# godk1122/IsaacLab

Hardware: AMD Instinct MI355X
Metric: env-steps/sec (whole node), Anymal-C rough 4096 envs/GPU, RSL-RL PPO iteration (collect+GAE+update) (higher is better)
Workload: dtype f32; 1 GPU; Isaac-Velocity-Rough-Anymal-C-v0, 4096 envs/GPU, T=24, 5 epochs x 4 minibatches, terrain 1204008 triangles, 4 state snapshots resident in HBM; parallelism=dp1, rollout=hipGraph, full_step=False, update=hipGraph (measured eager 16.24 ms, graph 15.60 ms), policy_params=571801

## Files before the change

### include/imx.h

```cpp
#ifndef IMX_H_
#define IMX_H_

#include <stddef.h>
#include <stdint.h>

#ifdef __cplusplus
extern "C" {
#endif

typedef struct imx_plan imx_plan_t;
typedef struct imx_mesh imx_mesh_t;
typedef void* imx_stream_t;

#define IMX_MAGIC 0x31584D49
#define IMX_PLAN_VERSION 3
#define IMX_HEADER_WORDS 48
#define IMX_MAX_OBS_GROUPS 4
#define IMX_REC_WORDS 20
#define IMX_FRAME_WORDS 9
#define IMX_FT_HEADER_WORDS 4

enum imx_header_word {
    IMX_H_MAGIC = 0, IMX_H_VERSION, IMX_H_J, IMX_H_B, IMX_H_H, IMX_H_A, IMX_H_D, IMX_H_R, IMX_H_NTERM, IMX_H_NREW,
    IMX_H_NOBS, IMX_H_NACT, IMX_H_MAX_EP_LEN, IMX_H_STEP_DT , IMX_H_TERM_OFF, IMX_H_REW_OFF, IMX_H_OBS_OFF,
// ... 514 lines not shown
size_t imx_empirical_normalization_partials_bytes(int64_t N, int64_t D);
int imx_empirical_normalization_update(int ngroups, const imx_norm_group_t* groups, imx_stream_t stream);


size_t imx_mlp_scratch_bytes(int64_t M, int out_features, int in_features);

int imx_mlp_dw(int64_t M, int N, int K, const float* dY_d, int64_t ldy, const float* X_d, int64_t ldx, float* dW_d,
               float* db_d, void* scratch_d, size_t scratch_bytes, imx_stream_t stream);

typedef struct imx_reduce_batch imx_reduce_batch_t;
int imx_reduce_batch_create(imx_reduce_batch_t** out);
void imx_reduce_batch_destroy(imx_reduce_batch_t* batch);
int imx_mlp_set_dw_cu_budget(int cus);
int imx_reduce_batch_begin(imx_reduce_batch_t* batch);
int imx_reduce_batch_flush(imx_reduce_batch_t* batch, imx_stream_t stream);

int imx_mlp_dw_elu(int64_t M, int N, int K, const float* dH_d, int64_t ldg, const float* H_d, int64_t ldh, float elu_alpha,
                   float* dZ_out_d, int64_t ldd, const float* X_d, int64_t ldx, float* dW_d, float* db_d, void* scratch_d,
                   size_t scratch_bytes, imx_stream_t stream);

int imx_mlp_infer(int64_t M, const float* X_d, int64_t ldx, int nnets, const int* nlayers, const int* dims,
                  const float* const* weights_d, const int* weight_pitch, const float* const* biases_d, const float* elu_alpha,
                  float* const* out_d, imx_stream_t stream);

typedef struct imx_policy_act {
    const float* std_d;
    uint64_t seed;
    const int32_t* step_counter_d;
    float* actions_out_d;
    float* logp_out_d;
    float* mu_out_d;
    float* sigma_out_d;
    float* obs_out_d;
    const imx_plan_t* plan;
// ... 126 lines not shown
```

### isaaclab_amd/csrc/mlp.hip

```cpp
#include <algorithm>

#include "imx_internal.h"
#include "imx_infer_device.h"


namespace {

constexpr int DW_T = 128;
constexpr int DW_BM = 32;
constexpr int DW_LD = DW_T + 32;

struct DwArgs {
    int64_t M;
    int N, K;
    const float* dY;
    int64_t ldy;
    const float* X;
    int64_t ldx;
    float* part;
    float* part_db;
    int tn, tk, S;
    int64_t rps;
    const float* H;
    int64_t ldh;
    float* Dout;
    int64_t ldd;
    float alpha;
};

template <bool VEC>
__device__ __forceinline__ void dw_load(float (&r)[16], const float* __restrict__ src, int64_t ld, int64_t row0, int64_t row_end,
                                        int col0, int ncols, int t) {
    if (VEC) {
        const int c = col0 + 4 * (t & 31);
        const int rr = t >> 5;
#pragma unroll
        for (int i = 0; i < 4; ++i) {
            const int64_t row = row0 + rr + 8 * i;
            float4 v = make_float4(0.f, 0.f, 0.f, 0.f);
            if (row < row_end && c < ncols) v = *reinterpret_cast<const float4*>(src + row * ld + c);
            r[4 * i] = v.x; r[4 * i + 1] = v.y; r[4 * i + 2] = v.z; r[4 * i + 3] = v.w;
        }
    } else {
        const int c = col0 + (t & 127);
        const int rr = t >> 7;
#pragma unroll
        for (int i = 0; i < 16; ++i) {
            const int64_t row = row0 + rr + 2 * i;
            r[i] = (row < row_end && c < ncols) ? src[row * ld + c] : 0.0f;
        }
    }
}

template <bool VEC>
__device__ __forceinline__ void dw_store(const float (&r)[16], float* __restrict__ s, int t) {
    if (VEC) {
        const int c = 4 * (t & 31), rr = t >> 5;
#pragma unroll
        for (int i = 0; i < 4; ++i)
            *reinterpret_cast<float4*>(s + (rr + 8 * i) * DW_LD + c) = make_float4(r[4 * i], r[4 * i + 1], r[4 * i + 2], r[4 * i + 3]);
    } else {
        const int c = t & 127, rr = t >> 7;
#pragma unroll
        for (int i = 0; i < 16; ++i) s[(rr + 2 * i) * DW_LD + c] = r[i];
    }
}

template <bool VEC>
__device__ __forceinline__ void dw_store_global(const float (&r)[16], float* __restrict__ dst, int64_t ld, int64_t row0, int64_t row_end,
                                                int col0, int ncols, int t, unsigned groups) {
    if (VEC) {
        const int c = col0 + 4 * (t & 31);
#pragma unroll
        for (int i = 0; i < 4; ++i) {
            const int64_t row = row0 + (t >> 5) + 8 * i;
            if (((groups >> i) & 1u) && row < row_end && c < ncols)
                *reinterpret_cast<float4*>(dst + row * ld + c) = make_float4(r[4 * i], r[4 * i + 1], r[4 * i + 2], r[4 * i + 3]);
        }
    } else {
// ... 1 lines not shown
#pragma unroll
        for (int i = 0; i < 16; ++i) {
            const int64_t row = row0 + (t >> 7) + 2 * i;
            if (row < row_end && c < ncols) dst[row * ld + c] = r[i];
        }
    }
}

typedef float dw_f4 __attribute__((ext_vector_type(4)));
typedef unsigned dw_u4 __attribute__((ext_vector_type(4)));

__device__ __forceinline__ __amdgpu_buffer_rsrc_t dw_rsrc(const float* p, int64_t rows, int64_t ld, int ncols) {
    return __builtin_amdgcn_make_buffer_rsrc(const_cast<float*>(p), 0, (int)(((rows - 1) * ld + ncols) * 4), 0x00020000);
}

template <bool ACT>
__device__ __forceinline__ void dw_movers_steady(const DwArgs& a, float* __restrict__ sY, float* __restrict__ sX, int t, int n0, int k0,
                                                 int64_t m_begin, int nst, bool want_db, unsigned dgroups, float (&dbv)[4]) {
    const int cl = 4 * (t & 31), rr = t >> 5;
    const int kv = (a.K + 3) & ~3;
    const int rows = nst * DW_BM;
    const int oy = (int)((rr * a.ldy + min(n0 + cl, a.N - 4)) * 4);
    const int ox = (int)((rr * a.ldx + min(k0 + cl, kv - 4)) * 4);
    const int oh = ACT ? (int)((rr * a.ldh + min(n0 + cl, a.N - 4)) * 4) : 0;
    const int od = ACT ? (int)((rr * a.ldd + n0 + cl) * 4) : 0;
    const bool d_ok = n0 + cl < a.N;
    const __amdgpu_buffer_rsrc_t by = dw_rsrc(a.dY + m_begin * a.ldy, rows, a.ldy, a.N);
    const __amdgpu_buffer_rsrc_t bx = dw_rsrc(a.X + m_begin * a.ldx, rows, a.ldx, kv);
    const __amdgpu_buffer_rsrc_t bh = dw_rsrc(ACT ? a.H + m_begin * a.ldh : a.dY, rows, ACT ? a.ldh : a.ldy, a.N);
    const __amdgpu_buffer_rsrc_t bd = dw_rsrc(ACT && dgroups != 0u ? a.Dout + m_begin * a.ldd : a.dY, rows, ACT ? a.ldd : a.ldy, a.N);
    const int gy = (int)(32 * a.ldy), gx = (int)(32 * a.ldx), gh = (int)(32 * a.ldh), gd = (int)(32 * a.ldd);
    int sy = 0, sx = 0, sh = 0, sd = 0;
    dw_f4 ry[4], rx[4], rh[ACT ? 4 : 1];
    auto load = [&]() __attribute__((always_inline)) {
#pragma unroll
        for (int i = 0; i < 4; ++i) ry[i] = __builtin_bit_cast(dw_f4, __builtin_amdgcn_raw_buffer_load_b128(by, oy, sy + i * gy, 0));
        if constexpr (ACT) {
#pragma unroll
            for (int i = 0; i < 4; ++i) rh[i] = __builtin_bit_cast(dw_f4, __builtin_amdgcn_raw_buffer_load_b128(bh, oh, sh + i * gh, 0));
            sh += 4 * gh;
        }
#pragma unroll
        for (int i = 0; i < 4; ++i) rx[i] = __builtin_bit_cast(dw_f4, __builtin_amdgcn_raw_buffer_load_b128(bx, ox, sx + i * gx, 0));
        sy += 4 * gy;
        sx += 4 * gx;
    };
    auto store = [&](int buf) __attribute__((always_inline)) {
        if constexpr (ACT) {
#pragma unroll
            for (int i = 0; i < 4; ++i)
#pragma unroll
                for (int j = 0; j < 4; ++j) ry[i][j] *= rh[i][j] > 0.0f ? 1.0f : rh[i][j] + a.alpha;
            if (dgroups != 0u) {
                if (d_ok) {
#pragma unroll
                    for (int i = 0; i < 4; ++i)
                        if ((dgroups >> i) & 1u) __builtin_amdgcn_raw_buffer_store_b128(__builtin_bit_cast(dw_u4, ry[i]), bd, od, sd + i * gd, 0);
                }
                sd += 4 * gd;
            }
        }
        float* py = sY + buf * (DW_BM * DW_LD) + rr * DW_LD + cl;
        float* px = sX + buf * (DW_BM * DW_LD) + rr * DW_LD + cl;
#pragma unroll
        for (int i = 0; i < 4; ++i) *reinterpret_cast<dw_f4*>(py + 8 * i * DW_LD) = ry[i];
#pragma unroll
        for (int i = 0; i < 4; ++i) *reinterpret_cast<dw_f4*>(px + 8 * i * DW_LD) = rx[i];
        if (want_db) {
#pragma unroll
            for (int i = 0; i < 4; ++i) { dbv[0] += ry[i][0]; dbv[1] += ry[i][1]; dbv[2] += ry[i][2]; dbv[3] += ry[i][3]; }
        }
    };
    load();
    store(0);
    if (nst > 1) load();
    __syncthreads();
    for (int st = 0; st < nst; ++st) {
        if (st + 1 < nst) {
            store((st + 1) & 1);
            if (st + 2 < nst) load();
        }
        __syncthreads();
    }
}

template <bool YVEC, bool XVEC, bool ACT>
__global__ void __launch_bounds__(512, 1) k_mlp_dw(DwArgs a) {
    __shared__ float sY[2][DW_BM * DW_LD];
    __shared__ float sX[2][DW_BM * DW_LD];
    const int T = a.tn * a.tk;
    int tile, s;
    if ((a.S & 7) == 0) {
        const int xcd = blockIdx.x & 7, j = blockIdx.x >> 3;
        tile = j % T;
        s = (j / T) * 8 + xcd;
    } else {
        tile = blockIdx.x % T;
        s = blockIdx.x / T;
    }
    const int n0 = (tile / a.tk) * DW_T, k0 = (tile % a.tk) * DW_T;
    const int64_t m_begin = (int64_t)s * a.rps, m_end = std::min<int64_t>(m_begin + a.rps, a.M);
    const int nst = (int)((m_end - m_begin + DW_BM - 1) / DW_BM);
    const bool want_db = a.part_db != nullptr && (tile % a.tk) == 0;

    if (threadIdx.x >= 256) {
        const int t = threadIdx.x - 256;
        float ry[16], rx[16], rh[ACT ? 16 : 1];
        float dbv[4] = {0.f, 0.f, 0.f, 0.f};
        int64_t loaded_row0 = 0;
        unsigned dgroups = 0u;
        if (ACT && a.Dout != nullptr) {
            if (YVEC) {
#pragma unroll
                for (int i = 0; i < 4; ++i) dgroups |= (i % a.tk) == (tile % a.tk) ? 1u << i : 0u;
            } else if ((tile % a.tk) == 0) {
                dgroups = 15u;
            }
        }
        const bool write_d = dgroups != 0u;
        bool steady = false;
        if constexpr (YVEC && XVEC) {
            int64_t ld = std::max(a.ldy, a.ldx);
            if (ACT) ld = std::max(ld, std::max(a.ldh, a.ldd));
            steady = nst > 0 && (m_end - m_begin) % DW_BM == 0 && a.rps * ld < ((int64_t)1 << 28);
            if (steady) dw_movers_steady<ACT>(a, &sY[0][0], &sX[0][0], t, n0, k0, m_begin, nst, want_db, dgroups, dbv);
        }
        auto load = [&](int st) {
            const int64_t row0 = m_begin + (int64_t)st * DW_BM;
            loaded_row0 = row0;
            dw_load<YVEC>(ry, a.dY, a.ldy, row0, m_end, n0, a.N, t);
            if constexpr (ACT) dw_load<YVEC>(rh, a.H, a.ldh, row0, m_end, n0, a.N, t);
            dw_load<XVEC>(rx, a.X, a.ldx, row0, m_end, k0, a.K, t);
        };
        auto store = [&](int buf) {
            if constexpr (ACT) {
#pragma unroll
                for (int q = 0; q < 16; ++q) ry[q] *= rh[q] > 0.0f ? 1.0f : rh[q] + a.alpha;
                if (write_d) dw_store_global<YVEC>(ry, a.Dout, a.ldd, loaded_row0, m_end, n0, a.N, t, dgroups);
            }
            dw_store<YVEC>(ry, sY[buf], t);
            dw_store<XVEC>(rx, sX[buf], t);
            if (want_db) {
                if (YVEC) {
#pragma unroll
                    for (int i = 0; i < 4; ++i) { dbv[0] += ry[4 * i]; dbv[1] += ry[4 * i + 1]; dbv[2] += ry[4 * i + 2]; dbv[3] += ry[4 * i + 3]; }
                } else {
#pragma unroll
                    for (int i = 0; i < 16; ++i) dbv[0] += ry[i];
                }
            }
        };
        if (!steady) {
            if (nst > 0) {
                load(0);
                store(0);
                if (nst > 1) load(1);
// ... 17 lines not shown
            }
        }
        __syncthreads();
        if (want_db && t < DW_T && n0 + t < a.N) {
            const float* red = sY[0];
            float sum = 0.0f;
            const int groups = YVEC ? 8 : 2;
            for (int g = 0; g < groups; ++g) sum += red[g * DW_T + t];
            a.part_db[(size_t)s * a.N + n0 + t] = sum;
        }
        return;
    }
    const int t = threadIdx.x;
    const int lane = t & 63, w = t >> 6, r = lane & 31, half = lane >> 5;
    const int wn = w & 1, wk = w >> 1;
    f32x16 acc[2][2];
#pragma unroll
    for (int i = 0; i < 2; ++i)
#pragma unroll
        for (int j = 0; j < 2; ++j)
#pragma unroll
            for (int q = 0; q < 16; ++q) acc[i][j][q] = 0.0f;
    __syncthreads();
    for (int st = 0; st < nst; ++st) {
        const float* py = sY[st & 1] + half * DW_LD + wn * 64 + r;
        const float* px = sX[st & 1] + half * DW_LD + wk * 64 + r;
        float p0 = py[0], p1 = py[32], p2 = px[0], p3 = px[32], q0, q1, q2, q3;
#pragma unroll
        for (int kk = 0; kk < DW_BM / 2; kk += 2) {
            q0 = py[(kk + 1) * 2 * DW_LD]; q1 = py[(kk + 1) * 2 * DW_LD + 32];
            q2 = px[(kk + 1) * 2 * DW_LD]; q3 = px[(kk + 1) * 2 * DW_LD + 32];
            __builtin_amdgcn_sched_barrier(0);
            acc[0][0] = __builtin_amdgcn_mfma_f32_32x32x2f32(p0, p2, acc[0][0], 0, 0, 0);
            acc[0][1] = __builtin_amdgcn_mfma_f32_32x32x2f32(p0, p3, acc[0][1], 0, 0, 0);
            acc[1][0] = __builtin_amdgcn_mfma_f32_32x32x2f32(p1, p2, acc[1][0], 0, 0, 0);
            acc[1][1] = __builtin_amdgcn_mfma_f32_32x32x2f32(p1, p3, acc[1][1], 0, 0, 0);
            __builtin_amdgcn_sched_barrier(0);
            if (kk + 2 < DW_BM / 2) {
                p0 = py[(kk + 2) * 2 * DW_LD]; p1 = py[(kk + 2) * 2 * DW_LD + 32];
                p2 = px[(kk + 2) * 2 * DW_LD]; p3 = px[(kk + 2) * 2 * DW_LD + 32];
            }
            __builtin_amdgcn_sched_barrier(0);
            acc[0][0] = __builtin_amdgcn_mfma_f32_32x32x2f32(q0, q2, acc[0][0], 0, 0, 0);
            acc[0][1] = __builtin_amdgcn_mfma_f32_32x32x2f32(q0, q3, acc[0][1], 0, 0, 0);
            acc[1][0] = __builtin_amdgcn_mfma_f32_32x32x2f32(q1, q2, acc[1][0], 0, 0, 0);
            acc[1][1] = __builtin_amdgcn_mfma_f32_32x32x2f32(q1, q3, acc[1][1], 0, 0, 0);
            __builtin_amdgcn_sched_barrier(0);
        }
        __syncthreads();
    }
    float* part = a.part + (size_t)s * a.N * a.K;
    const bool interior = n0 + DW_T <= a.N && k0 + DW_T <= a.K;
#pragma unroll
    for (int bi = 0; bi < 2; ++bi)
#pragma unroll
        for (int bj = 0; bj < 2; ++bj) {
            const int k = k0 + wk * 64 + bj * 32 + r;
            if (interior) {
#pragma unroll
                for (int q = 0; q < 16; ++q) part[(size_t)(n0 + wn * 64 + bi * 32 + acc_row(q, half)) * a.K + k] = acc[bi][bj][q];
            } else {
#pragma unroll
                for (int q = 0; q < 16; ++q) {
                    const int n = n0 + wn * 64 + bi * 32 + acc_row(q, half);
                    if (n < a.N && k < a.K) part[(size_t)n * a.K + k] = acc[bi][bj][q];
                }
            }
        }
    __syncthreads();
}

constexpr int RED_Y = 16;
__global__ void __launch_bounds__(64 * RED_Y) k_mlp_reduce(int64_t total, int S, const float* __restrict__ part, float* __restrict__ out,
                                                          int N, const float* __restrict__ part_db, float* __restrict__ db) {
    __shared__ float red[RED_Y][64];
    const int tx = threadIdx.x, ty = threadIdx.y;
    const int64_t i = (int64_t)blockIdx.x * 64 + tx;
    const float* src = nullptr;
    int64_t stride = 0;
    float* dst = nullptr;
    if (i < total) {
        src = part + i; stride = total; dst = out + i;
    } else if (db && i - total < N) {
        src = part_db + (i - total); stride = N; dst = db + (i - total);
// ... 78 lines not shown
        float sum = 0.0f;
#pragma unroll
        for (int y = 0; y < RED_Y; ++y) sum += red[y][tx];
        *dst = sum;
    }
}

struct DwPlan {
    int tn, tk, S;
    int64_t rps;
};

int g_num_cu = 0;
int g_dw_cu_budget = 0;

DwPlan dw_plan(int64_t M, int N, int K) {
    if (g_num_cu == 0) {
        int dev = 0, cu = 0;
        if (hipGetDevice(&dev) != hipSuccess || hipDeviceGetAttribute(&cu, hipDeviceAttributeMultiprocessorCount, dev) != hipSuccess || cu <= 0)
            cu = 256;
        g_num_cu = cu;
    }
    DwPlan p;
    p.tn = (N + DW_T - 1) / DW_T;
    p.tk = (K + DW_T - 1) / DW_T;
    const int T = p.tn * p.tk;
    const int cus = g_dw_cu_budget > 0 ? std::min(g_dw_cu_budget, g_num_cu) : g_num_cu;
    int64_t S = std::max<int64_t>(1, (int64_t)cus / T);
    S = std::min<int64_t>(S, std::max<int64_t>(1, M / (2 * DW_BM)));
    if (S >= 8) S &= ~(int64_t)7;
    p.rps = ((M + S - 1) / S + DW_BM - 1) / DW_BM * DW_BM;
    p.S = (int)((M + p.rps - 1) / p.rps);
    return p;
}

constexpr int HEAD_A = 64;

#define IMX_HALF_LOG_2PI_F 0.91893853320467274178f
template <bool ELU_IN, int AMAX, int LOSS>
__global__ void __launch_bounds__(256) k_head_fwd(int64_t M, int K, int A, float* __restrict__ h, int64_t ldh,
// ... 516 lines not shown
    return 0;
}

extern "C" void imx_reduce_batch_destroy(imx_reduce_batch_t* b) {
    if (t_batch == b) t_batch = nullptr;
    delete b;
}

extern "C" int imx_reduce_batch_begin(imx_reduce_batch_t* b) {
    IMX_REQUIRE(b, "imx_reduce_batch_begin: null batch");
    IMX_REQUIRE(t_batch == nullptr, "imx_reduce_batch_begin: another batch is still open on this thread (flush it first)");
    t_batch = b;
    return 0;
}

extern "C" int imx_reduce_batch_flush(imx_reduce_batch_t* b, imx_stream_t stream) {
    IMX_REQUIRE(b && t_batch == b, "imx_reduce_batch_flush: this batch is not the one open on this thread");
    t_batch = nullptr;
    if (b->args.n == 0) return 0;
    hipLaunchKernelGGL(k_mlp_reduce_batch, dim3(b->blocks), dim3(64, RED_Y), 0, (hipStream_t)stream, b->args);
    b->args.n = 0;
    b->blocks = 0;
    IMX_HIP(hipGetLastError());
    return 0;
}

extern "C" int imx_mlp_dw(int64_t M, int N, int K, const float* dY_d, int64_t ldy, const float* X_d, int64_t ldx, float* dW_d,
                          float* db_d, void* scratch_d, size_t scratch_bytes, imx_stream_t stream) {
    return mlp_dw_launch("imx_mlp_dw", M, N, K, dY_d, ldy, nullptr, 0, 0.0f, nullptr, 0, X_d, ldx, dW_d, db_d, scratch_d, scratch_bytes,
                         stream);
}

extern "C" int imx_mlp_dw_elu(int64_t M, int N, int K, const float* dH_d, int64_t ldg, const float* H_d, int64_t ldh, float elu_alpha,
                              float* dZ_out_d, int64_t ldd, const float* X_d, int64_t ldx, float* dW_d, float* db_d, void* scratch_d,
                              size_t scratch_bytes, imx_stream_t stream) {
    IMX_REQUIRE(H_d, "imx_mlp_dw_elu: the saved activation output is required");
    return mlp_dw_launch("imx_mlp_dw_elu", M, N, K, dH_d, ldg, H_d, ldh, elu_alpha, dZ_out_d, ldd, X_d, ldx, dW_d, db_d, scratch_d,
                         scratch_bytes, stream);
}

static int head_fwd_launch(int64_t M, int K, int A, float* h_d, int64_t ldh, const float* W_d, const float* b_d, float* y_d,
                           int elu_in_place, float elu_alpha, const imx_head_loss_t* loss, imx_stream_t stream) {
    IMX_REQUIRE(M > 0 && h_d && W_d && b_d && y_d, "imx_mlp_head_fwd: bad arguments");
    IMX_REQUIRE(A >= 1 && A <= HEAD_A, "imx_mlp_head_fwd: %d outputs (1..%d supported; wider layers are library GEMMs)", A, HEAD_A);
    IMX_REQUIRE(K >= 16 && K % 16 == 0 && K <= 2048 && ldh >= K && ldh % 4 == 0 && aligned16(h_d),
                "imx_mlp_head_fwd: in-features %d (pitch %lld) must be a multiple of 16, 16-byte aligned rows", K, (long long)ldh);
    IMX_REQUIRE((size_t)A * K * sizeof(float) <= 64 * 1024, "imx_mlp_head_fwd: %d x %d weights do not fit the 64 KB of LDS used", A, K);
    imx_head_loss_t L{};
    int mode = 0;
    if (loss) {
        L = *loss;
        mode = L.mode;
        IMX_REQUIRE(mode == 1 || mode == 2, "imx_mlp_head_fwd_loss: mode %d (1 policy, 2 value)", mode);
// ... 523 lines not shown
```

### isaaclab_amd/rsl_rl/ppo.py

```python

from __future__ import annotations

import ctypes
import os

import torch
import torch.distributed as dist
import torch.nn as nn
import torch.nn.functional as F

from .. import _lib
from .._lib import check, lib
from .storage import RolloutStorage


class _FusedPPOLoss(torch.autograd.Function):
    @staticmethod
    def forward(ctx, mu, sigma, value, actions, old_logp, old_mu, old_sigma, adv, ret, old_value, clip, clipped, vcoef, ecoef):
        L = lib()
        M, A = mu.shape
        mu_c, sg_c, v_c = mu.contiguous(), sigma.contiguous(), value.contiguous()
        args = [t.contiguous() for t in (actions, old_logp, old_mu, old_sigma, adv, ret, old_value)]
        actions, old_logp, old_mu, old_sigma, adv, ret, old_value = args
        out8 = torch.empty(8, device=mu.device)
# ... 187 lines not shown


HEAD_MAX_OUT = 64


def _is_head(lin: nn.Linear, x: torch.Tensor) -> bool:
    return (lin.out_features <= HEAD_MAX_OUT and lin.in_features % 32 == 0 and lin.in_features <= 256
            and x.stride(1) == 1 and x.stride(0) % 4 == 0)


FUSED_FIRST_LAYER_MAX_K = 256

FUSED_L0 = os.getenv("IMX_FUSED_L0", "1") != "0"
FUSED_HEAD = os.getenv("IMX_FUSED_HEAD", "0")
LOSS_ON_SIDE = os.getenv("IMX_LOSS_ON_SIDE", "1") == "1"


def fused_first_layer_ok(x: torch.Tensor, w: torch.Tensor) -> bool:
    return (x.is_cuda and x.dtype == torch.float32 and x.stride(1) == 1 and w.is_contiguous() and w.shape[1] == x.shape[1]
            and x.shape[1] <= FUSED_FIRST_LAYER_MAX_K and FUSED_L0)


def mlp_scratch(layers, M: int, device) -> torch.Tensor:
    n = max(int(lib().imx_mlp_scratch_bytes(M, lin.out_features, lin.in_features)) for lin, _ in layers)
    return torch.empty(n, dtype=torch.uint8, device=device)


class DeferredReductions:

    def __init__(self, layers, M: int, device):
# ... 80 lines not shown
                h = z
            else:
                h = F.elu(z, alpha=act.alpha, inplace=True)
            saved.append(h)
        else:
            h = act(z)
            saved.append((z, h))
    if pending_elu is not None:
        h = F.elu(h, alpha=pending_elu, inplace=True)
    if out is not None and h is not out:
        out.copy_(h)
        h = out
    return h, saved


def mlp_backward(layers, saved, dout, scratch=None, head_dprev=None):
    L = lib()
    M = dout.shape[0]
    if scratch is None:
        scratch = mlp_scratch(layers, M, dout.device)
    stream = _lib.current_stream(dout.device)
    deferred = scratch if isinstance(scratch, DeferredReductions) else None
    if deferred is not None:
        check(L.imx_reduce_batch_begin(deferred.handle))
    try:
        _mlp_backward_layers(L, layers, saved, dout, M, scratch, deferred, stream, head_dprev)
    finally:
        if deferred is not None:
            check(L.imx_reduce_batch_flush(deferred.handle, stream))


def _mlp_backward_layers(L, layers, saved, dout, M, scratch, deferred, stream, head_dprev=None):
    d = dout
    pending = None
    top = len(layers) - 1
    if head_dprev is not None:
        d, top = head_dprev, top - 1
    for i in range(top, -1, -1):
        lin, _ = layers[i]
        x = saved[i] if not isinstance(saved[i], tuple) else saved[i][1]
        prev_act = layers[i - 1][1] if i > 0 else None
        N, K = lin.out_features, lin.in_features
        scr = deferred.scratch[i] if deferred is not None else scratch
        if pending is not None:
            dh, h, alpha = pending
            pending = None
            d = torch.empty_like(dh) if i > 0 else None
            check(L.imx_mlp_dw_elu(M, N, K, dh.data_ptr(), dh.stride(0), h.data_ptr(), h.stride(0), float(alpha),
                                   _lib.ptr(d), N, x.data_ptr(), x.stride(0), lin.weight.grad.data_ptr(),
                                   lin.bias.grad.data_ptr(), scr.data_ptr(), scr.numel(), stream))
        else:
            if not d.is_contiguous():
                d = d.contiguous()
            if i > 0 and _is_head(lin, x) and (prev_act is None or isinstance(prev_act, nn.ELU)):
                dprev = torch.empty(M, K, device=d.device, dtype=d.dtype)
                check(L.imx_mlp_head_bwd(M, K, N, d.data_ptr(), x.data_ptr(), x.stride(0), lin.weight.data_ptr(),
                                         float(prev_act.alpha) if prev_act is not None else 0.0, int(prev_act is not None),
                                         dprev.data_ptr(), lin.weight.grad.data_ptr(), lin.bias.grad.data_ptr(),
                                         scr.data_ptr(), scr.numel(), stream))
                d = dprev
                continue
            check(L.imx_mlp_dw(M, N, K, d.data_ptr(), d.stride(0), x.data_ptr(), x.stride(0), lin.weight.grad.data_ptr(),
                               lin.bias.grad.data_ptr(), scr.data_ptr(), scr.numel(), stream))
        if i > 0:
            dx = torch.mm(d, lin.weight)
            if isinstance(prev_act, nn.ELU) and dx.stride(1) == 1 and saved[i].stride(1) == 1:
                pending = (dx, saved[i], prev_act.alpha)
            elif isinstance(prev_act, nn.ELU):
                d = torch.ops.aten.elu_backward(dx, prev_act.alpha, 1.0, 1.0, True, saved[i])
            elif prev_act is None:
                d = dx
            else:
                z, h = saved[i]
                d = _act_backward(prev_act, dx, z, h)


def _act_backward(act, dh, z, h):
    if isinstance(act, nn.Identity):
        return dh
    if isinstance(act, nn.Tanh):
# ... 214 lines not shown
        return self._side

    def _aux_stream(self):
        if getattr(self, "_aux", None) is None:
            self._aux = torch.cuda.Stream(self.device)
        return self._aux

    def _workspace(self, M: int, A: int):
        ws = self._ws.get((M, A))
        if ws is None:
            dev = self.device
            ws = dict(dmu=torch.empty(M, A, device=dev), dsigma=torch.empty(M, A, device=dev), dvalue=torch.empty(M, 1, device=dev),
                      scratch=torch.empty(int(lib().imx_ppo_scratch_bytes(M)), dtype=torch.uint8, device=dev),
                      colsum=torch.empty(int(lib().imx_colsum_scratch_bytes()), dtype=torch.uint8, device=dev),
                      mlp_a=DeferredReductions(self._actor_layers, M, dev), mlp_c=DeferredReductions(self._critic_layers, M, dev))
            self._ws[(M, A)] = ws
        return ws

    def minibatch_step(self, obs, critic_obs, actions, target_values, advantages, returns, old_logp, old_mu, old_sigma):
        L = lib()
        pol = self.policy
        stream = _lib.current_stream(self.device)
        M, A = actions.shape
        for name, t in (("actions", actions), ("target_values", target_values), ("advantages", advantages), ("returns", returns),
                        ("old_actions_log_prob", old_logp), ("old_mu", old_mu), ("old_sigma", old_sigma)):
            if not t.is_contiguous():
                raise _lib.ImxError(f"PPO.minibatch_step: {name} must be contiguous (shape {tuple(t.shape)}, strides {t.stride()})")
        ws = self._workspace(M, A)
        if pol.noise_std_type == "scalar":
            sigma, sstride = pol.std, 0
# ... 50 lines not shown
            else:
                torch.sum(ws["dsigma"] * sigma, dim=0, out=pol.log_std.grad)

        first_a = first_c = z0 = None
        joint_elu = None
        if self._joint0 is not None and critic_obs.data_ptr() == obs.data_ptr() and critic_obs.shape == obs.shape:
            w0, b0, H0, alpha0 = self._joint0
            if fused_first_layer_ok(obs, w0):
                z0 = torch.empty(obs.shape[0], 2 * H0, device=obs.device)
                check(L.imx_mlp_fwd_elu(obs.shape[0], 2 * H0, obs.shape[1], obs.data_ptr(), obs.stride(0), w0.data_ptr(), b0.data_ptr(),
                                        alpha0, 1, z0.data_ptr(), z0.stride(0), stream))
            else:
                z0 = torch.addmm(b0, obs, w0.t())
                joint_elu = alpha0
            first_a, first_c = z0[:, :H0], z0[:, H0:]
        side = self._side_stream()
        main = torch.cuda.current_stream(self.device)
        if side is not None:
            loss_on_side = LOSS_ON_SIDE
            aux = self._aux_stream()
            side.wait_stream(main)
            if joint_elu is not None:
                F.elu(first_a, alpha=joint_elu, inplace=True)
            mu, saved_a = actor_pass(stream)
            mu_ready = torch.cuda.Event()
            mu_ready.record(main)
            with torch.cuda.stream(side):
                if joint_elu is not None:
                    F.elu(first_c, alpha=joint_elu, inplace=True)
                value, saved_c = critic_pass(side.cuda_stream)
                value_ready = torch.cuda.Event()
                value_ready.record(side)
            if not loss_on_side:
                aux.wait_stream(main)
                aux.wait_event(value_ready)
            mlp_backward(self._actor_layers, saved_a, ws["dmu"], ws["mlp_a"], head_dprev=heads["a"])
            with torch.cuda.stream(side):
                mlp_backward(self._critic_layers, saved_c, ws["dvalue"], ws["mlp_c"], head_dprev=heads["c"])
                if loss_on_side:
                    side.wait_event(mu_ready)
                    loss_values(mu, value, side.cuda_stream)
            if not loss_on_side:
                with torch.cuda.stream(aux):
                    loss_values(mu, value, aux.cuda_stream)
            main.wait_stream(side)
            if not loss_on_side:
                main.wait_stream(aux)
            mu.record_stream(aux)
            mu.record_stream(side)
            value.record_stream(aux)
            value.record_stream(main)
            if z0 is not None:
                z0.record_stream(side)
        else:
            if joint_elu is not None:
                F.elu(z0, alpha=joint_elu, inplace=True)
            mu, saved_a = actor_pass(stream)
            value, saved_c = critic_pass(stream)
            loss_values(mu, value, stream)
            mlp_backward(self._actor_layers, saved_a, ws["dmu"], ws["mlp_a"], head_dprev=heads["a"])
            mlp_backward(self._critic_layers, saved_c, ws["dvalue"], ws["mlp_c"], head_dprev=heads["c"])
        return self._out8

    update_graph = False
    _update_calls = 0
    _update_g = None
    _update_t = None

    @torch.no_grad()
    def update(self):
        if not (self.update_graph and self.device.type == "cuda" and not self.is_multi_gpu) or self._update_t == "eager":
            return self._update_eager()
        self._update_calls += 1
        c = self._update_calls
        if c == 1:
            return self._update_eager()
# ... 72 lines not shown
```

Before: 5.466 million env-steps/s.

## Fuse actor and critic first-layer weight-gradient into one wide stacked dW kernel

Adds a wide dW kernel variant that covers two 128-column K tiles per block (WK=2) and reads dH from per-segment pointers. It uses this variant to compute the first-layer weight and bias gradients for the stacked actor and critic layer in a single launch. The per-network backward passes now stop above the first layer and return the first-layer input gradient, defer their reductions, and sync across streams before the joint dW launch. The aim is to cut launch count and reread fewer X tiles by reusing the observation tile across both networks. The cost is a larger LDS footprint, more registers, and a stream join that serialises the critic branch with the main stream.

```diff
diff --git a/include/imx.h b/include/imx.h
--- a/include/imx.h
+++ b/include/imx.h
@@ -552,10 +552,16 @@
 int imx_mlp_set_dw_cu_budget(int cus);
 int imx_reduce_batch_begin(imx_reduce_batch_t* batch);
 int imx_reduce_batch_flush(imx_reduce_batch_t* batch, imx_stream_t stream);
+int imx_reduce_batch_end(imx_reduce_batch_t* batch);
 
 int imx_mlp_dw_elu(int64_t M, int N, int K, const float* dH_d, int64_t ldg, const float* H_d, int64_t ldh, float elu_alpha,
                    float* dZ_out_d, int64_t ldd, const float* X_d, int64_t ldx, float* dW_d, float* db_d, void* scratch_d,
                    size_t scratch_bytes, imx_stream_t stream);
+
+size_t imx_mlp_dw_wide_scratch_bytes(int64_t M, int out_features, int in_features);
+int imx_mlp_dw_elu_wide(int64_t M, int N, int K, int n_seg, const float* const* dH_seg_d, int seg_cols, int64_t ldg, const float* H_d,
+                        int64_t ldh, float elu_alpha, const float* X_d, int64_t ldx, float* dW_d, float* db_d, void* scratch_d,
+                        size_t scratch_bytes, imx_reduce_batch_t* defer_to, imx_stream_t stream);
 
 int imx_mlp_infer(int64_t M, const float* X_d, int64_t ldx, int nnets, const int* nlayers, const int* dims,
                   const float* const* weights_d, const int* weight_pitch, const float* const* biases_d, const float* elu_alpha,
diff --git a/isaaclab_amd/csrc/mlp.hip b/isaaclab_amd/csrc/mlp.hip
--- a/isaaclab_amd/csrc/mlp.hip
+++ b/isaaclab_amd/csrc/mlp.hip
@@ -9,6 +9,8 @@
 constexpr int DW_T = 128;
 constexpr int DW_BM = 32;
 constexpr int DW_LD = DW_T + 32;
+constexpr int dw_ldx(int wk) { return DW_T * wk + 32; }
+constexpr int DW_MAX_SEG = 4;
 
 struct DwArgs {
     int64_t M;
@@ -27,6 +29,10 @@
     int64_t ldd;
     float alpha;
 };
+struct DwSeg {
+    int segw;
+    const float* yseg[DW_MAX_SEG];
+};
 
 template <bool VEC>
 __device__ __forceinline__ void dw_load(float (&r)[16], const float* __restrict__ src, int64_t ld, int64_t row0, int64_t row_end,
@@ -52,17 +58,17 @@
     }
 }
 
-template <bool VEC>
+template <bool VEC, int LD = DW_LD>
 __device__ __forceinline__ void dw_store(const float (&r)[16], float* __restrict__ s, int t) {
     if (VEC) {
         const int c = 4 * (t & 31), rr = t >> 5;
 #pragma unroll
         for (int i = 0; i < 4; ++i)
-            *reinterpret_cast<float4*>(s + (rr + 8 * i) * DW_LD + c) = make_float4(r[4 * i], r[4 * i + 1], r[4 * i + 2], r[4 * i + 3]);
+            *reinterpret_cast<float4*>(s + (rr + 8 * i) * LD + c) = make_float4(r[4 * i], r[4 * i + 1], r[4 * i + 2], r[4 * i + 3]);
     } else {
         const int c = t & 127, rr = t >> 7;
 #pragma unroll
-        for (int i = 0; i < 16; ++i) s[(rr + 2 * i) * DW_LD + c] = r[i];
+        for (int i = 0; i < 16; ++i) s[(rr + 2 * i) * LD + c] = r[i];
     }
 }
 
@@ -94,24 +100,28 @@
     return __builtin_amdgcn_make_buffer_rsrc(const_cast<float*>(p), 0, (int)(((rows - 1) * ld + ncols) * 4), 0x00020000);
 }
 
-template <bool ACT>
-__device__ __forceinline__ void dw_movers_steady(const DwArgs& a, float* __restrict__ sY, float* __restrict__ sX, int t, int n0, int k0,
-                                                 int64_t m_begin, int nst, bool want_db, unsigned dgroups, float (&dbv)[4]) {
+template <bool ACT, int WK>
+__device__ __forceinline__ void dw_movers_steady(const DwArgs& a, const float* __restrict__ dYb, int yn0, int yN, float* __restrict__ sY,
+                                                 float* __restrict__ sX, int t, int n0, int k0, int64_t m_begin, int nst, bool want_db,
+                                                 unsigned dgroups, float (&dbv)[4]) {
+    constexpr int LDX = dw_ldx(WK);
     const int cl = 4 * (t & 31), rr = t >> 5;
     const int kv = (a.K + 3) & ~3;
     const int rows = nst * DW_BM;
-    const int oy = (int)((rr * a.ldy + min(n0 + cl, a.N - 4)) * 4);
-    const int ox = (int)((rr * a.ldx + min(k0 + cl, kv - 4)) * 4);
+    const int oy = (int)((rr * a.ldy + min(yn0 + cl, yN - 4)) * 4);
+    int ox[WK];
+#pragma unroll
+    for (int h = 0; h < WK; ++h) ox[h] = (int)((rr * a.ldx + min(k0 + h * DW_T + cl, kv - 4)) * 4);
     const int oh = ACT ? (int)((rr * a.ldh + min(n0 + cl, a.N - 4)) * 4) : 0;
     const int od = ACT ? (int)((rr * a.ldd + n0 + cl) * 4) : 0;
     const bool d_ok = n0 + cl < a.N;
-    const __amdgpu_buffer_rsrc_t by = dw_rsrc(a.dY + m_begin * a.ldy, rows, a.ldy, a.N);
+    const __amdgpu_buffer_rsrc_t by = dw_rsrc(dYb + m_begin * a.ldy, rows, a.ldy, yN);
     const __amdgpu_buffer_rsrc_t bx = dw_rsrc(a.X + m_begin * a.ldx, rows, a.ldx, kv);
     const __amdgpu_buffer_rsrc_t bh = dw_rsrc(ACT ? a.H + m_begin * a.ldh : a.dY, rows, ACT ? a.ldh : a.ldy, a.N);
     const __amdgpu_buffer_rsrc_t bd = dw_rsrc(ACT && dgroups != 0u ? a.Dout + m_begin * a.ldd : a.dY, rows, ACT ? a.ldd : a.ldy, a.N);
     const int gy = (int)(32 * a.ldy), gx = (int)(32 * a.ldx), gh = (int)(32 * a.ldh), gd = (int)(32 * a.ldd);
     int sy = 0, sx = 0, sh = 0, sd = 0;
-    dw_f4 ry[4], rx[4], rh[ACT ? 4 : 1];
+    dw_f4 ry[4], rx[WK][4], rh[ACT ? 4 : 1];
     auto load = [&]() __attribute__((always_inline)) {
 #pragma unroll
         for (int i = 0; i < 4; ++i) ry[i] = __builtin_bit_cast(dw_f4, __builtin_amdgcn_raw_buffer_load_b128(by, oy, sy + i * gy, 0));
@@ -121,7 +131,9 @@
             sh += 4 * gh;
         }
 #pragma unroll
-        for (int i = 0; i < 4; ++i) rx[i] = __builtin_bit_cast(dw_f4, __builtin_amdgcn_raw_buffer_load_b128(bx, ox, sx + i * gx, 0));
+        for (int h = 0; h < WK; ++h)
+#pragma unroll
+            for (int i = 0; i < 4; ++i) rx[h][i] = __builtin_bit_cast(dw_f4, __builtin_amdgcn_raw_buffer_load_b128(bx, ox[h], sx + i * gx, 0));
         sy += 4 * gy;
         sx += 4 * gx;
     };
@@ -141,11 +153,13 @@
             }
         }
         float* py = sY + buf * (DW_BM * DW_LD) + rr * DW_LD + cl;
-        float* px = sX + buf * (DW_BM * DW_LD) + rr * DW_LD + cl;
+        float* px = sX + buf * (DW_BM * LDX) + rr * LDX + cl;
 #pragma unroll
         for (int i = 0; i < 4; ++i) *reinterpret_cast<dw_f4*>(py + 8 * i * DW_LD) = ry[i];
 #pragma unroll
-        for (int i = 0; i < 4; ++i) *reinterpret_cast<dw_f4*>(px + 8 * i * DW_LD) = rx[i];
+        for (int h = 0; h < WK; ++h)
+#pragma unroll
+            for (int i = 0; i < 4; ++i) *reinterpret_cast<dw_f4*>(px + h * DW_T + 8 * i * LDX) = rx[h][i];
         if (want_db) {
 #pragma unroll
             for (int i = 0; i < 4; ++i) { dbv[0] += ry[i][0]; dbv[1] += ry[i][1]; dbv[2] += ry[i][2]; dbv[3] += ry[i][3]; }
@@ -164,10 +178,11 @@
     }
 }
 
-template <bool YVEC, bool XVEC, bool ACT>
-__global__ void __launch_bounds__(512, 1) k_mlp_dw(DwArgs a) {
+template <bool YVEC, bool XVEC, bool ACT, int WK>
+__device__ __forceinline__ void dw_tile(const DwArgs& a, const DwSeg& g) {
+    constexpr int LDX = dw_ldx(WK), DW_TK = DW_T * WK;
     __shared__ float sY[2][DW_BM * DW_LD];
-    __shared__ float sX[2][DW_BM * DW_LD];
+    __shared__ float sX[2][DW_BM * LDX];
     const int T = a.tn * a.tk;
     int tile, s;
     if ((a.S & 7) == 0) {
@@ -178,14 +193,24 @@
         tile = blockIdx.x % T;
         s = blockIdx.x / T;
     }
-    const int n0 = (tile / a.tk) * DW_T, k0 = (tile % a.tk) * DW_T;
+    const int n0 = (tile / a.tk) * DW_T, k0 = (tile % a.tk) * DW_TK;
+    const float* dYb = a.dY;
+    int yn0 = n0, yN = a.N;
+    if constexpr (WK == 2) {
+        if (g.segw > 0) {
+            const int sg = n0 / g.segw;
+            dYb = sg == 0 ? g.yseg[0] : sg == 1 ? g.yseg[1] : sg == 2 ? g.yseg[2] : g.yseg[3];
+            yn0 = n0 - sg * g.segw;
+            yN = min(g.segw, a.N - sg * g.segw);
+        }
+    }
     const int64_t m_begin = (int64_t)s * a.rps, m_end = std::min<int64_t>(m_begin + a.rps, a.M);
     const int nst = (int)((m_end - m_begin + DW_BM - 1) / DW_BM);
     const bool want_db = a.part_db != nullptr && (tile % a.tk) == 0;
 
     if (threadIdx.x >= 256) {
         const int t = threadIdx.x - 256;
-        float ry[16], rx[16], rh[ACT ? 16 : 1];
+        float ry[16], rx[WK][16], rh[ACT ? 16 : 1];
         float dbv[4] = {0.f, 0.f, 0.f, 0.f};
         int64_t loaded_row0 = 0;
         unsigned dgroups = 0u;
@@ -203,14 +228,15 @@
             int64_t ld = std::max(a.ldy, a.ldx);
             if (ACT) ld = std::max(ld, std::max(a.ldh, a.ldd));
             steady = nst > 0 && (m_end - m_begin) % DW_BM == 0 && a.rps * ld < ((int64_t)1 << 28);
-            if (steady) dw_movers_steady<ACT>(a, &sY[0][0], &sX[0][0], t, n0, k0, m_begin, nst, want_db, dgroups, dbv);
+            if (steady) dw_movers_steady<ACT, WK>(a, dYb, yn0, yN, &sY[0][0], &sX[0][0], t, n0, k0, m_begin, nst, want_db, dgroups, dbv);
         }
         auto load = [&](int st) {
             const int64_t row0 = m_begin + (int64_t)st * DW_BM;
             loaded_row0 = row0;
-            dw_load<YVEC>(ry, a.dY, a.ldy, row0, m_end, n0, a.N, t);
+            dw_load<YVEC>(ry, dYb, a.ldy, row0, m_end, yn0, yN, t);
             if constexpr (ACT) dw_load<YVEC>(rh, a.H, a.ldh, row0, m_end, n0, a.N, t);
-            dw_load<XVEC>(rx, a.X, a.ldx, row0, m_end, k0, a.K, t);
+            dw_load<XVEC>(rx[0], a.X, a.ldx, row0, m_end, k0, a.K, t);
+            if constexpr (WK == 2) dw_load<XVEC>(rx[1], a.X, a.ldx, row0, m_end, k0 + DW_T, a.K, t);
         };
         auto store = [&](int buf) {
             if constexpr (ACT) {
@@ -219,7 +245,8 @@
                 if (write_d) dw_store_global<YVEC>(ry, a.Dout, a.ldd, loaded_row0, m_end, n0, a.N, t, dgroups);
             }
             dw_store<YVEC>(ry, sY[buf], t);
-            dw_store<XVEC>(rx, sX[buf], t);
+            dw_store<XVEC, LDX>(rx[0], sX[buf], t);
+            if constexpr (WK == 2) dw_store<XVEC, LDX>(rx[1], sX[buf] + DW_T, t);
             if (want_db) {
                 if (YVEC) {
 #pragma unroll
@@ -267,49 +294,88 @@
     const int t = threadIdx.x;
     const int lane = t & 63, w = t >> 6, r = lane & 31, half = lane >> 5;
     const int wn = w & 1, wk = w >> 1;
-    f32x16 acc[2][2];
+    constexpr int NBK = 2 * WK;
+    f32x16 acc[2][NBK];
 #pragma unroll
     for (int i = 0; i < 2; ++i)
 #pragma unroll
-        for (int j = 0; j < 2; ++j)
+        for (int j = 0; j < NBK; ++j)
 #pragma unroll
             for (int q = 0; q < 16; ++q) acc[i][j][q] = 0.0f;
     __syncthreads();
-    for (int st = 0; st < nst; ++st) {
-        const float* py = sY[st & 1] + half * DW_LD + wn * 64 + r;
-        const float* px = sX[st & 1] + half * DW_LD + wk * 64 + r;
-        float p0 = py[0], p1 = py[32], p2 = px[0], p3 = px[32], q0, q1, q2, q3;
-#pragma unroll
-        for (int kk = 0; kk < DW_BM / 2; kk += 2) {
-            q0 = py[(kk + 1) * 2 * DW_LD]; q1 = py[(kk + 1) * 2 * DW_LD + 32];
-            q2 = px[(kk + 1) * 2 * DW_LD]; q3 = px[(kk + 1) * 2 * DW_LD + 32];
-            __builtin_amdgcn_sched_barrier(0);
-            acc[0][0] = __builtin_amdgcn_mfma_f32_32x32x2f32(p0, p2, acc[0][0], 0, 0, 0);
-            acc[0][1] = __builtin_amdgcn_mfma_f32_32x32x2f32(p0, p3, acc[0][1], 0, 0, 0);
-            acc[1][0] = __builtin_amdgcn_mfma_f32_32x32x2f32(p1, p2, acc[1][0], 0, 0, 0);
-            acc[1][1] = __builtin_amdgcn_mfma_f32_32x32x2f32(p1, p3, acc[1][1], 0, 0, 0);
-            __builtin_amdgcn_sched_barrier(0);
-            if (kk + 2 < DW_BM / 2) {
-                p0 = py[(kk + 2) * 2 * DW_LD]; p1 = py[(kk + 2) * 2 * DW_LD + 32];
-                p2 = px[(kk + 2) * 2 * DW_LD]; p3 = px[(kk + 2) * 2 * DW_LD + 32];
-            }
-            __builtin_amdgcn_sched_barrier(0);
-            acc[0][0] = __builtin_amdgcn_mfma_f32_32x32x2f32(q0, q2, acc[0][0], 0, 0, 0);
-            acc[0][1] = __builtin_amdgcn_mfma_f32_32x32x2f32(q0, q3, acc[0][1], 0, 0, 0);
-            acc[1][0] = __builtin_amdgcn_mfma_f32_32x32x2f32(q1, q2, acc[1][0], 0, 0, 0);
-            acc[1][1] = __builtin_amdgcn_mfma_f32_32x32x2f32(q1, q3, acc[1][1], 0, 0, 0);
-            __builtin_amdgcn_sched_barrier(0);
-        }
-        __syncthreads();
+    if constexpr (WK == 2) {
+        for (int st = 0; st < nst; ++st) {
+            const float* py = sY[st & 1] + half * DW_LD + wn * 64 + r;
+            const float* px = sX[st & 1] + half * LDX + wk * 128 + r;
+            float p0 = py[0], p1 = py[32], p2 = px[0], p3 = px[32], p4 = px[64], p5 = px[96], q0, q1, q2, q3, q4, q5;
+#pragma unroll
+            for (int kk = 0; kk < DW_BM / 2; kk += 2) {
+                q0 = py[(kk + 1) * 2 * DW_LD]; q1 = py[(kk + 1) * 2 * DW_LD + 32];
+                q2 = px[(kk + 1) * 2 * LDX]; q3 = px[(kk + 1) * 2 * LDX + 32]; q4 = px[(kk + 1) * 2 * LDX + 64]; q5 = px[(kk + 1) * 2 * LDX + 96];
+                __builtin_amdgcn_sched_barrier(0);
+                acc[0][0] = __builtin_amdgcn_mfma_f32_32x32x2f32(p0, p2, acc[0][0], 0, 0, 0);
+                acc[0][1] = __builtin_amdgcn_mfma_f32_32x32x2f32(p0, p3, acc[0][1], 0, 0, 0);
+                acc[0][2] = __builtin_amdgcn_mfma_f32_32x32x2f32(p0, p4, acc[0][2], 0, 0, 0);
+                acc[0][3] = __builtin_amdgcn_mfma_f32_32x32x2f32(p0, p5, acc[0][3], 0, 0, 0);
+                acc[1][0] = __builtin_amdgcn_mfma_f32_32x32x2f32(p1, p2, acc[1][0], 0, 0, 0);
+                acc[1][1] = __builtin_amdgcn_mfma_f32_32x32x2f32(p1, p3, acc[1][1], 0, 0, 0);
+                acc[1][2] = __builtin_amdgcn_mfma_f32_32x32x2f32(p1, p4, acc[1][2], 0, 0, 0);
+                acc[1][3] = __builtin_amdgcn_mfma_f32_32x32x2f32(p1, p5, acc[1][3], 0, 0, 0);
+                __builtin_amdgcn_sched_barrier(0);
+                if (kk + 2 < DW_BM / 2) {
+                    p0 = py[(kk + 2) * 2 * DW_LD]; p1 = py[(kk + 2) * 2 * DW_LD + 32];
+                    p2 = px[(kk + 2) * 2 * LDX]; p3 = px[(kk + 2) * 2 * LDX + 32]; p4 = px[(kk + 2) * 2 * LDX + 64]; p5 = px[(kk + 2) * 2 * LDX + 96];
+                }
+                __builtin_amdgcn_sched_barrier(0);
+                acc[0][0] = __builtin_amdgcn_mfma_f32_32x32x2f32(q0, q2, acc[0][0], 0, 0, 0);
+                acc[0][1] = __builtin_amdgcn_mfma_f32_32x32x2f32(q0, q3, acc[0][1], 0, 0, 0);
+                acc[0][2] = __builtin_amdgcn_mfma_f32_32x32x2f32(q0, q4, acc[0][2], 0, 0, 0);
+                acc[0][3] = __builtin_amdgcn_mfma_f32_32x32x2f32(q0, q5, acc[0][3], 0, 0, 0);
+                acc[1][0] = __builtin_amdgcn_mfma_f32_32x32x2f32(q1, q2, acc[1][0], 0, 0, 0);
+                acc[1][1] = __builtin_amdgcn_mfma_f32_32x32x2f32(q1, q3, acc[1][1], 0, 0, 0);
+                acc[1][2] = __builtin_amdgcn_mfma_f32_32x32x2f32(q1, q4, acc[1][2], 0, 0, 0);
+                acc[1][3] = __builtin_amdgcn_mfma_f32_32x32x2f32(q1, q5, acc[1][3], 0, 0, 0);
+                __builtin_amdgcn_sched_barrier(0);
+            }
+            __syncthreads();
+        }
+    } else {
+        for (int st = 0; st < nst; ++st) {
+            const float* py = sY[st & 1] + half * DW_LD + wn * 64 + r;
+            const float* px = sX[st & 1] + half * DW_LD + wk * 64 + r;
+            float p0 = py[0], p1 = py[32], p2 = px[0], p3 = px[32], q0, q1, q2, q3;
+#pragma unroll
+            for (int kk = 0; kk < DW_BM / 2; kk += 2) {
+                q0 = py[(kk + 1) * 2 * DW_LD]; q1 = py[(kk + 1) * 2 * DW_LD + 32];
+                q2 = px[(kk + 1) * 2 * DW_LD]; q3 = px[(kk + 1) * 2 * DW_LD + 32];
+                __builtin_amdgcn_sched_barrier(0);
+                acc[0][0] = __builtin_amdgcn_mfma_f32_32x32x2f32(p0, p2, acc[0][0], 0, 0, 0);
+                acc[0][1] = __builtin_amdgcn_mfma_f32_32x32x2f32(p0, p3, acc[0][1], 0, 0, 0);
+                acc[1][0] = __builtin_amdgcn_mfma_f32_32x32x2f32(p1, p2, acc[1][0], 0, 0, 0);
+                acc[1][1] = __builtin_amdgcn_mfma_f32_32x32x2f32(p1, p3, acc[1][1], 0, 0, 0);
+                __builtin_amdgcn_sched_barrier(0);
+                if (kk + 2 < DW_BM / 2) {
+                    p0 = py[(kk + 2) * 2 * DW_LD]; p1 = py[(kk + 2) * 2 * DW_LD + 32];
+                    p2 = px[(kk + 2) * 2 * DW_LD]; p3 = px[(kk + 2) * 2 * DW_LD + 32];
+                }
+                __builtin_amdgcn_sched_barrier(0);
+                acc[0][0] = __builtin_amdgcn_mfma_f32_32x32x2f32(q0, q2, acc[0][0], 0, 0, 0);
+                acc[0][1] = __builtin_amdgcn_mfma_f32_32x32x2f32(q0, q3, acc[0][1], 0, 0, 0);
+                acc[1][0] = __builtin_amdgcn_mfma_f32_32x32x2f32(q1, q2, acc[1][0], 0, 0, 0);
+                acc[1][1] = __builtin_amdgcn_mfma_f32_32x32x2f32(q1, q3, acc[1][1], 0, 0, 0);
+                __builtin_amdgcn_sched_barrier(0);
+            }
+            __syncthreads();
+        }
     }
     float* part = a.part + (size_t)s * a.N * a.K;
-    const bool interior = n0 + DW_T <= a.N && k0 + DW_T <= a.K;
+    const bool interior = n0 + DW_T <= a.N && k0 + DW_TK <= a.K;
 #pragma unroll
     for (int bi = 0; bi < 2; ++bi)
 #pragma unroll
-        for (int bj = 0; bj < 2; ++bj) {
-            const int k = k0 + wk * 64 + bj * 32 + r;
-            if (interior) {
+        for (int bj = 0; bj < NBK; ++bj) {
+            const int k = k0 + wk * (32 * NBK) + bj * 32 + r;
+            if (WK == 2 ? (n0 + DW_T <= a.N && k0 + wk * (32 * NBK) + bj * 32 + 32 <= a.K) : interior) {
 #pragma unroll
                 for (int q = 0; q < 16; ++q) part[(size_t)(n0 + wn * 64 + bi * 32 + acc_row(q, half)) * a.K + k] = acc[bi][bj][q];
             } else {
@@ -321,6 +387,16 @@
             }
         }
     __syncthreads();
+}
+
+template <bool YVEC, bool XVEC, bool ACT>
+__global__ void __launch_bounds__(512, 1) k_mlp_dw(DwArgs a) {
+    dw_tile<YVEC, XVEC, ACT, 1>(a, DwSeg{});
+}
+
+template <bool YVEC, bool XVEC, bool ACT>
+__global__ void __launch_bounds__(512, 1) k_mlp_dw_wide(DwArgs a, DwSeg g) {
+    dw_tile<YVEC, XVEC, ACT, 2>(a, g);
 }
 
 constexpr int RED_Y = 16;
@@ -429,7 +505,7 @@
 int g_num_cu = 0;
 int g_dw_cu_budget = 0;
 
-DwPlan dw_plan(int64_t M, int N, int K) {
+DwPlan dw_plan(int64_t M, int N, int K, bool wide = false) {
     if (g_num_cu == 0) {
         int dev = 0, cu = 0;
         if (hipGetDevice(&dev) != hipSuccess || hipDeviceGetAttribute(&cu, hipDeviceAttributeMultiprocessorCount, dev) != hipSuccess || cu <= 0)
@@ -438,7 +514,7 @@
     }
     DwPlan p;
     p.tn = (N + DW_T - 1) / DW_T;
-    p.tk = (K + DW_T - 1) / DW_T;
+    p.tk = wide ? 1 : (K + DW_T - 1) / DW_T;
     const int T = p.tn * p.tk;
     const int cus = g_dw_cu_budget > 0 ? std::min(g_dw_cu_budget, g_num_cu) : g_num_cu;
     int64_t S = std::max<int64_t>(1, (int64_t)cus / T);
@@ -985,6 +1061,12 @@
     return 0;
 }
 
+extern "C" int imx_reduce_batch_end(imx_reduce_batch_t* b) {
+    IMX_REQUIRE(b && t_batch == b, "imx_reduce_batch_end: this batch is not the one open on this thread");
+    t_batch = nullptr;
+    return 0;
+}
+
 extern "C" int imx_reduce_batch_flush(imx_reduce_batch_t* b, imx_stream_t stream) {
     IMX_REQUIRE(b && t_batch == b, "imx_reduce_batch_flush: this batch is not the one open on this thread");
     t_batch = nullptr;
@@ -1008,6 +1090,57 @@
     IMX_REQUIRE(H_d, "imx_mlp_dw_elu: the saved activation output is required");
     return mlp_dw_launch("imx_mlp_dw_elu", M, N, K, dH_d, ldg, H_d, ldh, elu_alpha, dZ_out_d, ldd, X_d, ldx, dW_d, db_d, scratch_d,
                          scratch_bytes, stream);
+}
+
+extern "C" size_t imx_mlp_dw_wide_scratch_bytes(int64_t M, int out_features, int in_features) {
+    if (M <= 0 || out_features <= 0 || in_features <= DW_T || in_features > 2 * DW_T) return 0;
+    const DwPlan p = dw_plan(M, out_features, in_features, true);
+    return ((size_t)p.S * out_features * in_features + (size_t)p.S * out_features) * sizeof(float) + 256;
+}
+
+extern "C" int imx_mlp_dw_elu_wide(int64_t M, int N, int K, int n_seg, const float* const* dH_seg_d, int seg_cols, int64_t ldg,
+                                   const float* H_d, int64_t ldh, float elu_alpha, const float* X_d, int64_t ldx, float* dW_d, float* db_d,
+                                   void* scratch_d, size_t scratch_bytes, imx_reduce_batch_t* defer_to, imx_stream_t stream) {
+    const char* who = "imx_mlp_dw_elu_wide";
+    IMX_REQUIRE(M > 0 && N > 0 && dH_seg_d && H_d && X_d && dW_d && scratch_d, "%s: bad arguments", who);
+    IMX_REQUIRE(K > DW_T && K <= 2 * DW_T, "%s: %d in-features (the 128 x 256 tile serves 129..256; imx_mlp_dw_elu serves the rest)", who, K);
+    IMX_REQUIRE(n_seg >= 1 && n_seg <= DW_MAX_SEG, "%s: %d gradient segments (1..%d)", who, n_seg, DW_MAX_SEG);
+    IMX_REQUIRE(n_seg == 1 ? seg_cols >= N : (seg_cols % DW_T == 0 && (int64_t)(n_seg - 1) * seg_cols < N && (int64_t)n_seg * seg_cols >= N),
+                "%s: %d segments of %d columns do not cover %d out-features in whole 128-row slabs", who, n_seg, seg_cols, N);
+    for (int i = 0; i < n_seg; ++i) IMX_REQUIRE(dH_seg_d[i], "%s: gradient segment %d is null", who, i);
+    const int widest = n_seg == 1 ? N : seg_cols;
+    IMX_REQUIRE(ldg >= widest && ldh >= N && ldx >= K, "%s: row pitch smaller than the row (ldg=%lld, ldh=%lld N=%d, ldx=%lld K=%d)", who,
+                (long long)ldg, (long long)ldh, N, (long long)ldx, K);
+    const DwPlan p = dw_plan(M, N, K, true);
+    const size_t need = ((size_t)p.S * N * K + (size_t)p.S * N) * sizeof(float);
+    IMX_REQUIRE(scratch_bytes >= need, "%s: scratch too small (%zu < %zu bytes; see imx_mlp_dw_wide_scratch_bytes)", who, scratch_bytes, need);
+    DwArgs a;
+    a.M = M; a.N = N; a.K = K;
+    a.dY = dH_seg_d[0]; a.ldy = ldg; a.X = X_d; a.ldx = ldx;
+    a.part = (float*)scratch_d;
+    a.part_db = db_d ? a.part + (size_t)p.S * N * K : nullptr;
+    a.tn = p.tn; a.tk = p.tk; a.S = p.S; a.rps = p.rps;
+    a.H = H_d; a.ldh = ldh; a.Dout = nullptr; a.ldd = 0; a.alpha = elu_alpha;
+    DwSeg g;
+    g.segw = n_seg > 1 ? seg_cols : 0;
+    bool yvec = (N % 4 == 0) && (ldg % 4 == 0) && (ldh % 4 == 0) && aligned16(H_d);
+    for (int i = 0; i < DW_MAX_SEG; ++i) {
+        g.yseg[i] = i < n_seg ? dH_seg_d[i] : nullptr;
+        if (i < n_seg) yvec = yvec && aligned16(dH_seg_d[i]);
+    }
+    const bool xvec = (ldx % 4 == 0) && aligned16(X_d) && (K % 4 == 0 || ldx >= ((K + 3) & ~3));
+    const dim3 grid((unsigned)(p.tn * p.tk * p.S)), block(512);
+    hipStream_t st = (hipStream_t)stream;
+    if (yvec && xvec) hipLaunchKernelGGL((k_mlp_dw_wide<true, true, true>), grid, block, 0, st, a, g);
+    else if (yvec) hipLaunchKernelGGL((k_mlp_dw_wide<true, false, true>), grid, block, 0, st, a, g);
+    else if (xvec) hipLaunchKernelGGL((k_mlp_dw_wide<false, true, true>), grid, block, 0, st, a, g);
+    else hipLaunchKernelGGL((k_mlp_dw_wide<false, false, true>), grid, block, 0, st, a, g);
+    IMX_HIP(hipGetLastError());
+    imx_reduce_batch* saved = t_batch;
+    t_batch = defer_to;
+    const int rc = reduce_or_defer(who, (int64_t)N * K, p.S, a.part, dW_d, N, a.part_db, db_d, st);
+    t_batch = saved;
+    return rc;
 }
 
 static int head_fwd_launch(int64_t M, int K, int A, float* h_d, int64_t ldh, const float* W_d, const float* b_d, float* y_d,
diff --git a/isaaclab_amd/rsl_rl/ppo.py b/isaaclab_amd/rsl_rl/ppo.py
--- a/isaaclab_amd/rsl_rl/ppo.py
+++ b/isaaclab_amd/rsl_rl/ppo.py
@@ -225,6 +225,7 @@
 FUSED_L0 = os.getenv("IMX_FUSED_L0", "1") != "0"
 FUSED_HEAD = os.getenv("IMX_FUSED_HEAD", "0")
 LOSS_ON_SIDE = os.getenv("IMX_LOSS_ON_SIDE", "1") == "1"
+WIDE_DW0 = os.getenv("IMX_WIDE_DW0", "1") != "0"
 
 
 def fused_first_layer_ok(x: torch.Tensor, w: torch.Tensor) -> bool:
@@ -335,7 +336,7 @@
     return h, saved
 
 
-def mlp_backward(layers, saved, dout, scratch=None, head_dprev=None):
+def mlp_backward(layers, saved, dout, scratch=None, head_dprev=None, stop_above_first=False, flush=True):
     L = lib()
     M = dout.shape[0]
     if scratch is None:
@@ -345,19 +346,32 @@
     if deferred is not None:
         check(L.imx_reduce_batch_begin(deferred.handle))
     try:
-        _mlp_backward_layers(L, layers, saved, dout, M, scratch, deferred, stream, head_dprev)
+        return _mlp_backward_layers(L, layers, saved, dout, M, scratch, deferred, stream, head_dprev, 1 if stop_above_first else 0)
     finally:
-        if deferred is not None:
+        if deferred is not None and flush:
             check(L.imx_reduce_batch_flush(deferred.handle, stream))
-
-
-def _mlp_backward_layers(L, layers, saved, dout, M, scratch, deferred, stream, head_dprev=None):
+        elif deferred is not None:
+            check(L.imx_reduce_batch_end(deferred.handle))
+
+
+def wide_dw0_ok(layers, x: torch.Tensor) -> bool:
+    if len(layers) < 2 or not isinstance(layers[0][1], nn.ELU):
+        return False
+    lin0, lin1 = layers[0][0], layers[1][0]
+    if not 128 < lin0.in_features <= 256 or lin0.out_features % 128 != 0:
+        return False
+    if lin1.out_features <= HEAD_MAX_OUT and lin1.in_features % 32 == 0 and lin1.in_features <= 256:
+        return False
+    return x.dtype == torch.float32 and x.stride(1) == 1 and x.stride(0) % 4 == 0 and x.data_ptr() % 16 == 0
+
+
+def _mlp_backward_layers(L, layers, saved, dout, M, scratch, deferred, stream, head_dprev=None, lowest=0):
     d = dout
     pending = None
     top = len(layers) - 1
     if head_dprev is not None:
         d, top = head_dprev, top - 1
-    for i in range(top, -1, -1):
+    for i in range(top, lowest - 1, -1):
         lin, _ = layers[i]
         x = saved[i] if not isinstance(saved[i], tuple) else saved[i][1]
         prev_act = layers[i - 1][1] if i > 0 else None
@@ -385,6 +399,8 @@
                                lin.bias.grad.data_ptr(), scr.data_ptr(), scr.numel(), stream))
         if i > 0:
             dx = torch.mm(d, lin.weight)
+            if i == lowest:
+                return dx
             if isinstance(prev_act, nn.ELU) and dx.stride(1) == 1 and saved[i].stride(1) == 1:
                 pending = (dx, saved[i], prev_act.alpha)
             elif isinstance(prev_act, nn.ELU):
@@ -629,6 +645,10 @@
                       scratch=torch.empty(int(lib().imx_ppo_scratch_bytes(M)), dtype=torch.uint8, device=dev),
                       colsum=torch.empty(int(lib().imx_colsum_scratch_bytes()), dtype=torch.uint8, device=dev),
                       mlp_a=DeferredReductions(self._actor_layers, M, dev), mlp_c=DeferredReductions(self._critic_layers, M, dev))
+            if self._joint0 is not None and WIDE_DW0:
+                w0 = self._joint0[0]
+                n = int(lib().imx_mlp_dw_wide_scratch_bytes(M, w0.shape[0], w0.shape[1]))
+                ws["dw0"] = torch.empty(n, dtype=torch.uint8, device=dev) if n else None
             self._ws[(M, A)] = ws
         return ws
 
@@ -709,6 +729,22 @@
                 z0 = torch.addmm(b0, obs, w0.t())
                 joint_elu = alpha0
             first_a, first_c = z0[:, :H0], z0[:, H0:]
+        wide0 = (z0 is not None and ws.get("dw0") is not None and obs.shape[1] == self._joint0[0].shape[1]
+                 and wide_dw0_ok(self._actor_layers, obs) and wide_dw0_ok(self._critic_layers, obs))
+
+        def stacked_dw0(dh_a, dh_c, st):
+            w0, _b0, H0, alpha0 = self._joint0
+            la = self._actor_layers[0][0]
+            if dh_a.stride(0) != dh_c.stride(0) or dh_a.stride(1) != 1 or dh_c.stride(1) != 1:
+                raise _lib.ImxError("PPO.minibatch_step: the two first-layer gradients do not share a row pitch")
+            segs = (ctypes.c_void_p * 2)(dh_a.data_ptr(), dh_c.data_ptr())
+            batch = ws["mlp_a"].handle
+            check(L.imx_mlp_dw_elu_wide(M, 2 * H0, obs.shape[1], 2, segs, H0, dh_a.stride(0), z0.data_ptr(), z0.stride(0), alpha0,
+                                        obs.data_ptr(), obs.stride(0), la.weight.grad.data_ptr(), la.bias.grad.data_ptr(),
+                                        ws["dw0"].data_ptr(), ws["dw0"].numel(), batch, st))
+            check(L.imx_reduce_batch_begin(batch))
+            check(L.imx_reduce_batch_flush(batch, st))
+
         side = self._side_stream()
         main = torch.cuda.current_stream(self.device)
         if side is not None:
@@ -729,15 +765,26 @@
             if not loss_on_side:
                 aux.wait_stream(main)
                 aux.wait_event(value_ready)
-            mlp_backward(self._actor_layers, saved_a, ws["dmu"], ws["mlp_a"], head_dprev=heads["a"])
+            dh_a = mlp_backward(self._actor_layers, saved_a, ws["dmu"], ws["mlp_a"], head_dprev=heads["a"], stop_above_first=wide0,
+                                flush=not wide0)
             with torch.cuda.stream(side):
-                mlp_backward(self._critic_layers, saved_c, ws["dvalue"], ws["mlp_c"], head_dprev=heads["c"])
+                dh_c = mlp_backward(self._critic_layers, saved_c, ws["dvalue"], ws["mlp_c"], head_dprev=heads["c"], stop_above_first=wide0,
+                                    flush=not wide0)
+                if wide0:
+                    dh0_ready = torch.cuda.Event()
+                    dh0_ready.record(side)
+                    dh_c.record_stream(main)
+                    check(L.imx_reduce_batch_begin(ws["mlp_c"].handle))
+                    check(L.imx_reduce_batch_flush(ws["mlp_c"].handle, side.cuda_stream))
                 if loss_on_side:
                     side.wait_event(mu_ready)
                     loss_values(mu, value, side.cuda_stream)
             if not loss_on_side:
                 with torch.cuda.stream(aux):
                     loss_values(mu, value, aux.cuda_stream)
+            if wide0:
+                main.wait_event(dh0_ready)
+                stacked_dw0(dh_a, dh_c, stream)
             main.wait_stream(side)
             if not loss_on_side:
                 main.wait_stream(aux)
@@ -753,8 +800,11 @@
             mu, saved_a = actor_pass(stream)
             value, saved_c = critic_pass(stream)
             loss_values(mu, value, stream)
-            mlp_backward(self._actor_layers, saved_a, ws["dmu"], ws["mlp_a"], head_dprev=heads["a"])
-            mlp_backward(self._critic_layers, saved_c, ws["dvalue"], ws["mlp_c"], head_dprev=heads["c"])
+            dh_a = mlp_backward(self._actor_layers, saved_a, ws["dmu"], ws["mlp_a"], head_dprev=heads["a"], stop_above_first=wide0,
+                                flush=not wide0)
+            dh_c = mlp_backward(self._critic_layers, saved_c, ws["dvalue"], ws["mlp_c"], head_dprev=heads["c"], stop_above_first=wide0)
+            if wide0:
+                stacked_dw0(dh_a, dh_c, stream)
         return self._out8
 
     update_graph = False
```

Measured after the change: 5.607 million env-steps/s, median of 6. 2.6% higher.
